# rmcar17/SpectralClusterSupertree

Measured on NVIDIA B200. Metric: construct_supertree wall-time at 10k taxa/1k trees, lower is better.
Workload: dtype f64

## Files before the change

spectralclustersupertree_b200/csrc/common.cuh:

```cuda
#pragma once

#include <cuda_runtime.h>

#include <cstdint>
#include <cstdio>
#include <cstring>
#include <string>
#include <vector>

#include "scs_b200.h"

namespace scs {

constexpr int kMediumMaxDefault = 4096;

struct DeviceBuffer {
    void *ptr = nullptr;
    size_t bytes = 0;
};

enum Slot : int {
    SLOT_TOUR_OFFSETS = 0,
    SLOT_TOUR_TAXON,
    SLOT_TOUR_DEPTH,
// ... 223 lines not shown
int pcg_degree_block(scs_ctx *ctx, int n, int T, RowBlock rows, const double *W_block, double *degree);

int components(scs_ctx *ctx, int n, const uint32_t *bits, int32_t *label, int32_t *n_components_host);

int components_async(scs_ctx *ctx, int n, const uint32_t *bits, int32_t *label, int32_t *count_dev);

int contract(scs_ctx *ctx, int n, const double *W, const uint32_t *adj_bits, const uint32_t *max_bits,
             int32_t *group, int32_t *m_host, double *Wc, double *degree_c);
int contract_with_labels(scs_ctx *ctx, int n, const double *W, const uint32_t *adj_bits, const int32_t *label, int m,
                         int32_t *group, double *Wc, double *degree_c, RowBlock rows = RowBlock());

int spectral_bipartition(scs_ctx *ctx, int m, const double *W, const double *degree, uint64_t seed,
                         int32_t *side, scs_node_stats *stats_host, RowBlock rows = RowBlock());

int normalized_matvec(scs_ctx *ctx, int m, const double *W, const double *isd, const double *x, double *y);

int pcg_build_batch(scs_ctx *ctx, int B, int blocks, int R, int T, int64_t L, int max_n, int max_trees, const MedNode *nodes_dev,
                    const int32_t *tree_node, const int32_t *row_node, const int64_t *leaf_offsets,
                    const int32_t *leaf_taxon, const int32_t *adj_depth, const double *adj_val,
                    const int32_t *root_depth, const double *tree_weight, double *W, int32_t *occ, uint32_t *adj_bits,
                    uint32_t *max_bits, double *degree, int32_t *bad_dev);

constexpr int kMediumMax = kMediumMaxDefault;

int medium_batch(scs_ctx *ctx, int B, const int32_t *node_n, const int32_t *tree_begin, const int32_t *tree_end,
                 const int64_t *part_off, const uint64_t *seeds, int T, int64_t L, const int64_t *leaf_offsets, const int32_t *leaf_taxon,
                 const int32_t *adj_depth, const double *adj_val, const int32_t *root_depth, const double *tree_weight,
                 int contract_edges, int32_t *part_dev, scs_node_stats *stats_host, uint8_t *needs_rerun);

int small_node(scs_ctx *ctx, int n, int contract_edges, const double *W, const uint32_t *adj_bits,
               const uint32_t *max_bits, int32_t *part, scs_node_stats *out_dev, int32_t *group_out,
               double *Wc_out);

int small_batch(scs_ctx *ctx, int num_nodes, const scs_small_node *nodes_dev, const int64_t *leaf_offsets,
                const int32_t *leaf_taxon, const int32_t *adj_depth, const double *adj_val, const int32_t *root_depth,
                const double *tree_weight, int contract_edges, int32_t *part_dev, scs_node_stats *stats_dev,
                int32_t *bad_dev, int absolute_offsets = 0);

int small_cycles(scs_ctx *ctx, unsigned long long *out2, int reset);

int node_split(scs_ctx *ctx, int n, int T, int64_t L, const int64_t *leaf_offsets, const int32_t *leaf_taxon,
               const int32_t *adj_depth, const double *adj_val, const int32_t *root_depth,
               const double *tree_weight, int contract_edges, uint64_t seed, int32_t *part_dev,
               int32_t *part_host, scs_node_stats *stats);

bool shard_applies(const scs_ctx *ctx, int n);
int shard_barrier(scs_ctx *ctx);
int shard_push(scs_ctx *ctx, size_t offset, size_t bytes);
struct ShardMatvecTicket {
    unsigned long long epoch;
    size_t vec_offset;
    unsigned long long timeout_ns;
};
ShardMatvecTicket shard_next_matvec(scs_ctx *ctx);
int node_split_sharded(scs_ctx *ctx, int n, int T, int64_t L, const int64_t *leaf_offsets, const int32_t *leaf_taxon,
                       const int32_t *adj_depth, const double *adj_val, const int32_t *root_depth,
                       const double *tree_weight, int contract_edges, uint64_t seed, int32_t *part_dev,
                       int32_t *part_host, scs_node_stats *stats);

}
```

spectralclustersupertree_b200/csrc/devdriver.cu:

```cuda

#include "common.cuh"

#include <algorithm>
#include <chrono>
#include <cmath>
#include <cstdio>
#include <cstdlib>
#include <thread>

#include "devforest.cuh"
#include "driver.hpp"
#include "forest.hpp"

struct scs_device_forest {
    scs::DevForest trees;
    int weighting = 0;
    int num_taxa = 0;
    std::vector<int32_t> taxa;
    int64_t first_tree_nodes = 0, pair_visits = 0, leaves = 0;
    scs_ctx *owner = nullptr;
};

namespace scs {

// ... 361 lines not shown
                     std::vector<size_t> &reruns) {
        const DevForest &forest = current();
        const int B = static_cast<int>(medium.size());
        std::vector<int32_t> node_n(B), tree_begin(B), tree_end(B);
        std::vector<int64_t> part_off(B);
        std::vector<uint64_t> seeds(B);
        for (int b = 0; b < B; ++b) {
            const Job &job = wave[medium[b]];
            node_n[b] = static_cast<int32_t>(job.taxa.size());
            tree_begin[b] = job.where.tree_begin;
            tree_end[b] = job.where.tree_begin + job.where.trees;
            part_off[b] = splits[b].part_at;
            seeds[b] = node_seed(seed_, job.taxa[0], job.taxa.size());
        }
        std::vector<scs_node_stats> stats(B);
        std::vector<uint8_t> rerun(B, 0);
        int rc = medium_batch(ctx, B, node_n.data(), tree_begin.data(), tree_end.data(), part_off.data(), seeds.data(),
                              static_cast<int>(forest.trees), forest.leaves, forest.leaf_off.as<int64_t>(),
                              tours_.leaf_taxon.as<int32_t>(), tours_.adj_depth.as<int32_t>(), tours_.adj_val.as<double>(),
                              tours_.root_depth.as<int32_t>(), forest.weight.as<double>(), contract_, part_dev_.as<int32_t>(),
                              stats.data(), rerun.data());
        if (rc) return rc;
        for (int b = 0; b < B; ++b) {
            splits[b].stats = stats[b];
            if (rerun[b]) reruns.push_back(static_cast<size_t>(b));
        }
        return SCS_OK;
    }

    int split_small(scs_ctx *ctx, std::vector<Job> &wave, const std::vector<size_t> &small, Split *splits) {
        const DevForest &forest = current();
        const int B = static_cast<int>(small.size());
        std::vector<scs_small_node> desc(B);
        for (int b = 0; b < B; ++b) {
            const Job &job = wave[small[b]];
            desc[b].n = static_cast<int32_t>(job.taxa.size());
            desc[b].num_trees = job.where.trees;
            desc[b].leaf_base = job.where.leaf_begin;
            desc[b].tree_base = job.where.tree_begin;
            desc[b].vertex_base = splits[b].part_at;
        }
        int rc;
        const size_t bytes = sizeof(scs_small_node) * static_cast<size_t>(B);
        scs_small_node *desc_dev;
        if ((rc = reserve_as(ctx, SLOT_MED_NODES, static_cast<size_t>(B), &desc_dev))) return rc;
        void *pin_v;
        if ((rc = reserve_pinned(ctx, bytes + sizeof(scs_node_stats) * static_cast<size_t>(B) + 512, &pin_v))) return rc;
        unsigned char *pin = static_cast<unsigned char *>(pin_v);
        std::memcpy(pin, desc.data(), bytes);
        SCS_CUDA(ctx, cudaMemcpyAsync(desc_dev, pin, bytes, cudaMemcpyHostToDevice, ctx->stream));
        ctx->h2d_bytes += static_cast<int64_t>(bytes);
        scs_node_stats *stats_dev;
        if ((rc = reserve_as(ctx, SLOT_NODE_STATS, static_cast<size_t>(B), &stats_dev))) return rc;
        rc = small_batch(ctx, B, desc_dev, forest.leaf_off.as<int64_t>(), tours_.leaf_taxon.as<int32_t>(),
                         tours_.adj_depth.as<int32_t>(), tours_.adj_val.as<double>(), tours_.root_depth.as<int32_t>(),
                         forest.weight.as<double>(), contract_, part_dev_.as<int32_t>(), stats_dev, flags_dev_.as<int32_t>(), 1);
        if (rc) return rc;
        scs_node_stats *stats_pin = reinterpret_cast<scs_node_stats *>(pin + ((bytes + 255) & ~static_cast<size_t>(255)));
        SCS_CUDA(ctx, cudaMemcpyAsync(stats_pin, stats_dev, sizeof(scs_node_stats) * static_cast<size_t>(B), cudaMemcpyDeviceToHost,
                                       ctx->stream));
        SCS_CUDA(ctx, cudaStreamSynchronize(ctx->stream));
        ctx->d2h_bytes += static_cast<int64_t>(sizeof(scs_node_stats)) * B;
        for (int b = 0; b < B; ++b) splits[b].stats = stats_pin[b];
        return SCS_OK;
    }

    int plan_children(std::vector<Job> &wave, std::vector<Split> &splits, std::vector<Job> &next) {
        const int J = static_cast<int>(wave.size());
        std::vector<int32_t> job_tree_begin(static_cast<size_t>(J) + 1, 0), job_parts(J, 0), job_part_base(J, 0);
        for (int j = 0; j < J; ++j) job_tree_begin[j] = wave[j].where.tree_begin;
        job_tree_begin[J] = static_cast<int32_t>(current().trees);
        std::sort(splits.begin(), splits.end(), [](const Split &a, const Split &b) { return a.job < b.job; });
        struct Pending {
            int32_t parent_slot;
            bool parent_shared, stays;
            std::vector<int32_t> members;
        };
        std::vector<Pending> pending;
        std::vector<int32_t> part_newjob;
        std::vector<int32_t> start, members, cursor;
        for (Split &s : splits) {
            const Job &job = wave[s.job];
            const std::vector<int32_t> &taxa = job.taxa;
            const int n = static_cast<int>(taxa.size());
            const int parts = s.stats.n_components != 1 ? s.stats.n_components : 2;
            const int32_t *part = part_.data() + s.part_at;
            if (record_) {
// ... 195 lines not shown
```

spectralclustersupertree_b200/csrc/driver.cu:

```cuda

#include "common.cuh"

#include <algorithm>
#include <chrono>
#include <cstdio>
#include <cstdlib>
#include <cmath>
#include <memory>
#include <thread>

#include <omp.h>

#include "forest.hpp"
#include "driver.hpp"

namespace scs {

namespace {

constexpr int kMaxWorkers = 16;
int node_workers() {
    static const int value = [] {
        const char *env = std::getenv("SCS_NODE_WORKERS");
        const int v = env ? std::atoi(env) : 8;
// ... 68 lines not shown
    int32_t *tax() const { return reinterpret_cast<int32_t *>(base + o_tax); }
    int32_t *dep() const { return reinterpret_cast<int32_t *>(base + o_dep); }
    int32_t *root() const { return reinterpret_cast<int32_t *>(base + o_root); }
};

int small_stage(scs_ctx *ctx, int num_nodes, int64_t L_total, int64_t T_total, SmallStage *st) {
    const size_t nB = static_cast<size_t>(num_nodes), nL = static_cast<size_t>(L_total), nT = static_cast<size_t>(T_total);
    st->o_nodes = 0;
    st->o_off = st->o_nodes + nB * sizeof(scs_small_node);
    st->o_val = st->o_off + (nT + nB) * sizeof(int64_t);
    st->o_w = st->o_val + nL * sizeof(double);
    st->o_tax = st->o_w + nT * sizeof(double);
    st->o_dep = st->o_tax + nL * sizeof(int32_t);
    st->o_root = st->o_dep + nL * sizeof(int32_t);
    st->total = st->o_root + nT * sizeof(int32_t) + 64;
    if (ctx->pinned_io_bytes < st->total) {
        if (ctx->pinned_io) {
            SCS_CUDA(ctx, cudaStreamSynchronize(ctx->stream));
            SCS_CUDA(ctx, cudaFreeHost(ctx->pinned_io));
            ctx->pinned_io = nullptr;
            ctx->pinned_io_bytes = 0;
        }
        const size_t want = 2 * st->total + 4096;
        SCS_CUDA(ctx, cudaMallocHost(&ctx->pinned_io, want));
        ctx->pinned_io_bytes = want;
    }
    st->base = static_cast<unsigned char *>(ctx->pinned_io);
    return SCS_OK;
}

int small_run(scs_ctx *ctx, int num_nodes, const SmallStage &st, int contract_edges, int32_t *part,
              scs_node_stats *stats) {
    int64_t N_total = 0;
    const scs_small_node *nodes = st.nodes();
    for (int b = 0; b < num_nodes; ++b) {
        if (nodes[b].n < 1 || nodes[b].n > kSmallNode || nodes[b].num_trees < 0)
            return fail(ctx, SCS_ERR_INVALID, "small batch: node size out of range");
        if (nodes[b].num_trees > kSmallMaxTrees)
            return fail(ctx, SCS_ERR_INVALID, "small batch: more than 65 535 source trees at a node (use scs_node_split_*)");
        N_total += nodes[b].n;
    }
    const size_t nB = static_cast<size_t>(num_nodes);
    unsigned char *dev;
    int rc;
    if ((rc = reserve_as(ctx, SLOT_TOUR_OFFSETS, st.total, &dev))) return rc;
    SCS_CUDA(ctx, cudaMemcpyAsync(dev, st.base, st.total - 64, cudaMemcpyHostToDevice, ctx->stream));
    ctx->h2d_bytes += static_cast<int64_t>(st.total - 64);

    int32_t *part_dev, *bad_dev;
    scs_node_stats *stats_dev;
    if ((rc = reserve_as(ctx, SLOT_PART, static_cast<size_t>(N_total), &part_dev))) return rc;
    if ((rc = reserve_as(ctx, SLOT_NODE_STATS, nB, &stats_dev))) return rc;
    if ((rc = reserve_as(ctx, SLOT_SCALARS, 64, &bad_dev))) return rc;
    SCS_CUDA(ctx, cudaMemsetAsync(bad_dev, 0, sizeof(int32_t), ctx->stream));
    rc = small_batch(ctx, num_nodes, reinterpret_cast<const scs_small_node *>(dev + st.o_nodes),
                     reinterpret_cast<const int64_t *>(dev + st.o_off), reinterpret_cast<const int32_t *>(dev + st.o_tax),
                     reinterpret_cast<const int32_t *>(dev + st.o_dep), reinterpret_cast<const double *>(dev + st.o_val),
                     reinterpret_cast<const int32_t *>(dev + st.o_root), reinterpret_cast<const double *>(dev + st.o_w),
                     contract_edges, part_dev, stats_dev, bad_dev);
    if (rc) return rc;
    void *pin_v;
    if ((rc = reserve_pinned(ctx, 64, &pin_v))) return rc;
    SCS_CUDA(ctx, cudaMemcpyAsync(part, part_dev, sizeof(int32_t) * N_total, cudaMemcpyDeviceToHost, ctx->stream));
    SCS_CUDA(ctx, cudaMemcpyAsync(stats, stats_dev, sizeof(scs_node_stats) * nB, cudaMemcpyDeviceToHost, ctx->stream));
    SCS_CUDA(ctx, cudaMemcpyAsync(pin_v, bad_dev, sizeof(int32_t), cudaMemcpyDeviceToHost, ctx->stream));
    SCS_CUDA(ctx, cudaStreamSynchronize(ctx->stream));
    ctx->d2h_bytes += static_cast<int64_t>(sizeof(int32_t) * N_total + sizeof(scs_node_stats) * nB);
    if (*static_cast<int32_t *>(pin_v) != 0) return fail(ctx, SCS_ERR_INPUT, "leaf tour: taxon id out of range");
    for (int b = 0; b < num_nodes; ++b)
        if (stats[b].solver == -1) {
            stats[b].solver = 0;
            return fail(ctx, SCS_ERR_TOO_SMALL, "spectral step on a graph contracted to one vertex");
        }
    return SCS_OK;
}

class Driver {
  public:
    Driver(scs_ctx *ctx, int weighting, int contract_edges, uint64_t seed, bool record, int rank, int world,
           scs_supertree *out)
        : ctx_(ctx), weighting_(weighting), contract_(contract_edges), seed_(seed), record_(record), rank_(rank),
          world_(world), out_(*out) {}

    int run(const scs_forest *root) {
        num_taxa_ = scs_forest_num_taxa(root);
        scratch_.resize(static_cast<size_t>(std::max(scs_host_threads(), kMaxWorkers)));
        for (Scratch &sc : scratch_) sc.reset(num_taxa_);
        std::vector<Task> wave, next;
// ... 665 lines not shown
                               const int32_t *adj_depth, const double *adj_val, const int32_t *root_depth,
                               const double *tree_weight, int contract_edges, int32_t *part, scs_node_stats *stats) {
    if (!ctx || num_nodes < 0 || !nodes || !part || !stats || L_total < 0 || T_total < 0) return SCS_ERR_INVALID;
    if (num_nodes == 0) return SCS_OK;
    cudaSetDevice(ctx->device);
    SmallStage st;
    int rc = small_stage(ctx, num_nodes, L_total, T_total, &st);
    if (rc) return rc;
    const size_t nB = static_cast<size_t>(num_nodes), nL = static_cast<size_t>(L_total), nT = static_cast<size_t>(T_total);
    std::memcpy(st.nodes(), nodes, nB * sizeof(scs_small_node));
    std::memcpy(st.off(), leaf_offsets, (nT + nB) * sizeof(int64_t));
    if (nL) {
        std::memcpy(st.val(), adj_val, nL * sizeof(double));
        std::memcpy(st.tax(), leaf_taxon, nL * sizeof(int32_t));
        std::memcpy(st.dep(), adj_depth, nL * sizeof(int32_t));
    }
    if (nT) {
        std::memcpy(st.w(), tree_weight, nT * sizeof(double));
        std::memcpy(st.root(), root_depth, nT * sizeof(int32_t));
    }
    return small_run(ctx, num_nodes, st, contract_edges, part, stats);
}

int scs_nodes_split_small_dev(scs_ctx *ctx, int num_nodes, const scs_small_node *nodes_dev,
                              const int64_t *leaf_offsets_dev, const int32_t *leaf_taxon_dev,
                              const int32_t *adj_depth_dev, const double *adj_val_dev, const int32_t *root_depth_dev,
                              const double *tree_weight_dev, int contract_edges, int32_t *part_dev,
                              scs_node_stats *stats_dev) {
    if (!ctx || num_nodes < 0 || !nodes_dev || !part_dev || !stats_dev) return SCS_ERR_INVALID;
    cudaSetDevice(ctx->device);
    int32_t *bad_dev;
    int rc;
    if ((rc = reserve_as(ctx, SLOT_SCALARS, 64, &bad_dev))) return rc;
    return small_batch(ctx, num_nodes, nodes_dev, leaf_offsets_dev, leaf_taxon_dev, adj_depth_dev, adj_val_dev,
                       root_depth_dev, tree_weight_dev, contract_edges, part_dev, stats_dev, bad_dev);
}

int scs_supertree_build_sharded(scs_ctx *ctx, const scs_forest *forest, int weighting, int contract_edges,
                                uint64_t seed, int record_nodes, int rank, int world, scs_supertree **out) {
    if (!ctx || !forest || !out || weighting < 0 || weighting > 3 || world < 1 || rank < 0 || rank >= world)
        return SCS_ERR_INVALID;
    *out = nullptr;
    cudaSetDevice(ctx->device);
    std::unique_ptr<scs_supertree> result(new scs_supertree());
    int rc;
    const ShardState &sh = ctx->shard;
    const bool cooperative = world > 1 && sh.connected && sh.world == world && sh.rank == rank;
    if (ctx->device_forest && (world == 1 || cooperative)) {
        const scs_device_forest *resident = nullptr;
        const auto t0 = std::chrono::steady_clock::now();
        if ((rc = device_forest_refresh(ctx, forest, weighting, cooperative, &resident))) return rc;
        const auto t1 = std::chrono::steady_clock::now();
        rc = run_device_driver(ctx, resident, contract_edges, seed, record_nodes != 0, rank, world, result.get());
        const auto t2 = std::chrono::steady_clock::now();
        if (std::getenv("SCS_DRIVER_TRACE")) {
            auto ms = [](auto a, auto b) { return 1e3 * std::chrono::duration<double>(b - a).count(); };
            std::fprintf(stderr, "[scs build] rank %d: forest to the device %.2f ms, recursion %.2f ms, release %.2f ms\n", rank,
                         ms(t0, t1), ms(t1, t2), ms(t2, std::chrono::steady_clock::now()));
        }
    } else {
        Driver driver(ctx, weighting, contract_edges, seed, record_nodes != 0, rank, world, result.get());
        rc = driver.run(forest);
    }
    if (rc) return rc;
    if (world > 1 && result->shared_prefix == 0) result->shared_prefix = static_cast<int64_t>(result->parent.size());
    *out = result.release();
    return SCS_OK;
// ... 113 lines not shown
```

spectralclustersupertree_b200/csrc/pcg.cu:

```cuda

#include "common.cuh"

namespace scs {

namespace {

constexpr int kRowThreads = 512;
constexpr int kWarps = kRowThreads / 32;
constexpr size_t kRowsStaticSmem = 16 * 1024;

struct BatchView {
    const MedNode *nodes = nullptr;
    const int32_t *tree_node = nullptr;
    const int32_t *row_node = nullptr;
};

__global__ void pcg_index_leaves(int n, int T, int64_t L, const int64_t *__restrict__ leaf_offsets,
                                 const int32_t *__restrict__ leaf_taxon, int32_t *__restrict__ leaf_tree,
                                 int32_t *__restrict__ occ, int32_t *__restrict__ bad, BatchView batch) {
    int64_t g = blockIdx.x * static_cast<int64_t>(blockDim.x) + threadIdx.x;
    if (g >= L) return;
    int lo = 0, hi = T;
    while (hi - lo > 1) {
        int mid = (lo + hi) >> 1;
// ... 65 lines not shown

__global__ void pcg_sort_inverse(int row0, const int32_t *__restrict__ row_ptr, const int32_t *__restrict__ inv,
                                 int32_t *__restrict__ inv_sorted) {
    __shared__ int32_t stage[1024];
    const int a = row0 + blockIdx.x;
    const int base = row_ptr[a];
    const int cnt = row_ptr[a + 1] - base;
    for (int i0 = 0; i0 < cnt; i0 += blockDim.x) {
        const int i = i0 + threadIdx.x;
        const int32_t mine = i < cnt ? inv[base + i] : 0;
        int rank = 0;
        for (int j0 = 0; j0 < cnt; j0 += 1024) {
            const int len = min(1024, cnt - j0);
            __syncthreads();
            for (int j = threadIdx.x; j < len; j += blockDim.x) stage[j] = inv[base + j0 + j];
            __syncthreads();
            if (i < cnt)
                for (int j = 0; j < len; ++j) rank += stage[j] < mine;
        }
        if (i < cnt) inv_sorted[base + rank] = mine;
    }
}

struct __align__(16) LinkEntry {
    int32_t next_right, next_left;
    double val;
};
constexpr int32_t kNone = -1;
constexpr int32_t kRootLevel = -2;

__global__ void __launch_bounds__(256)
pcg_tour_links(int n, const int64_t *__restrict__ leaf_offsets, const int32_t *__restrict__ adj_depth,
               const double *__restrict__ adj_val, const int32_t *__restrict__ root_depth,
               LinkEntry *__restrict__ links) {
    extern __shared__ int32_t link_smem[];
    const int t = blockIdx.x;
    const int64_t tb = leaf_offsets[t];
    const int m = static_cast<int>(leaf_offsets[t + 1] - tb) - 1;
    if (m <= 0 || m >= n) return;
    const int32_t *D = adj_depth + tb;
    const int nb1 = (m + 31) >> 5, nb2 = (nb1 + 31) >> 5;
    int32_t *B1 = link_smem, *B2 = link_smem + nb1;
    const int lane = threadIdx.x & 31;
    for (int i0 = (threadIdx.x >> 5) << 5; i0 < m; i0 += blockDim.x) {
        int v = i0 + lane < m ? D[i0 + lane] : INT32_MAX;
#pragma unroll
        for (int off = 16; off > 0; off >>= 1) v = min(v, __shfl_xor_sync(0xffffffffu, v, off));
        if (lane == 0) B1[i0 >> 5] = v;
    }
    __syncthreads();
    for (int b0 = (threadIdx.x >> 5) << 5; b0 < nb1; b0 += blockDim.x) {
        int v = b0 + lane < nb1 ? B1[b0 + lane] : INT32_MAX;
#pragma unroll
        for (int off = 16; off > 0; off >>= 1) v = min(v, __shfl_xor_sync(0xffffffffu, v, off));
        if (lane == 0) B2[b0 >> 5] = v;
    }
    __syncthreads();
    const int rd = root_depth[t];
    for (int i = threadIdx.x; i < m; i += blockDim.x) {
        const int d = D[i];
        LinkEntry e;
        e.val = adj_val[tb + i];
        if (d == rd) {
            e.next_right = e.next_left = kRootLevel;
            links[tb + i] = e;
            continue;
        }
        int j = i + 1;
        {
// ... 957 lines not shown
    if ((rc = reserve_as(ctx, SLOT_LEAF_TREE, static_cast<size_t>(L) + 1, &leaf_tree))) return rc;
    if ((rc = reserve_as(ctx, SLOT_ROW_PTR, static_cast<size_t>(n) + 1, &row_ptr))) return rc;
    if ((rc = reserve_as(ctx, SLOT_CURSOR, static_cast<size_t>(n), &cursor))) return rc;
    if ((rc = reserve_as(ctx, SLOT_INV, static_cast<size_t>(L) + 1, &inv))) return rc;
    if ((rc = reserve_as(ctx, SLOT_INV_SORTED, static_cast<size_t>(L) + 1, &inv_sorted))) return rc;
    if ((rc = reserve_as(ctx, SLOT_SCALARS, 64, &scalars))) return rc;

    SCS_CUDA(ctx, cudaMemsetAsync(occ, 0, sizeof(int32_t) * n, ctx->stream));
    SCS_CUDA(ctx, cudaMemsetAsync(cursor, 0, sizeof(int32_t) * n, ctx->stream));
    SCS_CUDA(ctx, cudaMemsetAsync(scalars, 0, sizeof(int32_t) * 64, ctx->stream));
    if (L > 0) {
        pcg_index_leaves<<<ceil_div(L, 256), 256, 0, ctx->stream>>>(n, T, L, leaf_offsets, leaf_taxon, leaf_tree, occ,
                                                                   scalars, BatchView());
        SCS_LAUNCHED(ctx, "pcg_index_leaves");
    }
    if ((rc = exclusive_scan(ctx, n, occ, row_ptr))) return rc;
    if (L > 0) {
        pcg_fill_inverse<<<ceil_div(L, 256), 256, 0, ctx->stream>>>(n, L, leaf_taxon, leaf_tree, row_ptr, cursor, inv,
                                                                   BatchView());
        SCS_LAUNCHED(ctx, "pcg_fill_inverse");
        if (nrows > 0) {
            pcg_sort_inverse<<<nrows, 128, 0, ctx->stream>>>(row0, row_ptr, inv, inv_sorted);
            SCS_LAUNCHED(ctx, "pcg_sort_inverse");
        }
    }
    LinkEntry *links;
    if ((rc = reserve_as(ctx, SLOT_LINKS, static_cast<size_t>(L > 0 ? L : 1), &links))) return rc;
    if (L > 0 && T > 0) {
        const int nb1 = ceil_div(n, 32), nb2 = ceil_div(nb1, 32);
        const size_t link_smem = sizeof(int32_t) * (static_cast<size_t>(nb1) + nb2 + 2);
        if (link_smem > 48 * 1024)
            SCS_CUDA(ctx, cudaFuncSetAttribute(pcg_tour_links, cudaFuncAttributeMaxDynamicSharedMemorySize,
                                               static_cast<int>(link_smem)));
        pcg_tour_links<<<T, 256, link_smem, ctx->stream>>>(n, leaf_offsets, adj_depth, adj_val, root_depth, links);
        SCS_LAUNCHED(ctx, "pcg_tour_links");
    }

    const bool narrow = T < 65536;
    const size_t per_col = sizeof(double) + (narrow ? sizeof(uint16_t) : sizeof(int32_t));
    BucketShape bs;
    bs.warps_log2 = 4;
    const int warps = 1 << bs.warps_log2;
    bs.cols_per_chunk = chunk_columns(ctx, n, T);
    const int nchunks = ceil_div(n, bs.cols_per_chunk);
    bs.buckets = nchunks * warps;
    const int stride = ceil_div(bs.cols_per_chunk, warps) | 1;
    const size_t smem = static_cast<size_t>(stride) * warps * per_col + 16;
    if ((rc = reserve_as(ctx, SLOT_DEGREE_PART, static_cast<size_t>(n) * nchunks, &degree_part))) return rc;
    if (nrows == 0) return SCS_OK;

    const bool packed = n <= 65535 && !ctx->wide_entries;
    const size_t cells = static_cast<size_t>(T) * bs.buckets;
    if (cells + 1 >= (1ull << 31)) return fail(ctx, SCS_ERR_INVALID, "pcg_build: too many tree buckets");
    int32_t *bucket_ptr;
    void *entries;
    if ((rc = reserve_as(ctx, SLOT_BUCKET_PTR, cells + 2, &bucket_ptr))) return rc;
    if ((rc = reserve(ctx, SLOT_ENTRIES, (static_cast<size_t>(L) + 1) * (packed ? 4 : 8), &entries))) return rc;
    const bool tri = !rows.sharded() && C == nullptr && !ctx->full_rows;
    const bool half = rows.sharded() && rows.half_window && C == nullptr && !ctx->full_rows;
    int32_t *start16 = nullptr;
    if (tri && (rc = reserve_as(ctx, SLOT_START16, (static_cast<size_t>(L) + 1) * kWarps, &start16))) return rc;
    if ((rc = build_buckets(ctx, n, T, L, bs, stride, packed, leaf_offsets, leaf_taxon, bucket_ptr, entries, start16, scalars,
                            BatchView())))
        return rc;
    LeafStairs *stairs;
    if ((rc = reserve_as(ctx, SLOT_BUCKET_COUNT, static_cast<size_t>(L) + 1, &stairs))) return rc;
    if (L > 0) {
// ... 38 lines not shown
        !row_node || !W || !occ || !adj_bits || !degree || !bad_dev)
        return fail(ctx, SCS_ERR_INVALID, "pcg_build_batch: bad argument");
    BatchView batch;
    batch.nodes = nodes_dev;
    batch.tree_node = tree_node;
    batch.row_node = row_node;
    int32_t *leaf_tree, *row_ptr, *cursor, *inv, *inv_sorted;
    int rc;
    if ((rc = reserve_as(ctx, SLOT_LEAF_TREE, static_cast<size_t>(L) + 1, &leaf_tree))) return rc;
    if ((rc = reserve_as(ctx, SLOT_ROW_PTR, static_cast<size_t>(R) + 1, &row_ptr))) return rc;
    if ((rc = reserve_as(ctx, SLOT_CURSOR, static_cast<size_t>(R), &cursor))) return rc;
    if ((rc = reserve_as(ctx, SLOT_INV, static_cast<size_t>(L) + 1, &inv))) return rc;
    if ((rc = reserve_as(ctx, SLOT_INV_SORTED, static_cast<size_t>(L) + 1, &inv_sorted))) return rc;
    SCS_CUDA(ctx, cudaMemsetAsync(occ, 0, sizeof(int32_t) * R, ctx->stream));
    SCS_CUDA(ctx, cudaMemsetAsync(cursor, 0, sizeof(int32_t) * R, ctx->stream));
    if (L > 0) {
        pcg_index_leaves<<<ceil_div(L, 256), 256, 0, ctx->stream>>>(max_n, T, L, leaf_offsets, leaf_taxon, leaf_tree, occ,
                                                                   bad_dev, batch);
        SCS_LAUNCHED(ctx, "pcg_index_leaves");
    }
    if ((rc = exclusive_scan(ctx, R, occ, row_ptr))) return rc;
    if (L > 0) {
        pcg_fill_inverse<<<ceil_div(L, 256), 256, 0, ctx->stream>>>(max_n, L, leaf_taxon, leaf_tree, row_ptr, cursor, inv,
                                                                   batch);
        SCS_LAUNCHED(ctx, "pcg_fill_inverse");
        pcg_sort_inverse<<<R, 128, 0, ctx->stream>>>(0, row_ptr, inv, inv_sorted);
        SCS_LAUNCHED(ctx, "pcg_sort_inverse");
    }
    LinkEntry *links;
    if ((rc = reserve_as(ctx, SLOT_LINKS, static_cast<size_t>(L > 0 ? L : 1), &links))) return rc;
    if (L > 0 && T > 0) {
        const int nb1 = ceil_div(max_n + 1, 32), nb2 = ceil_div(nb1, 32);
        const size_t link_smem = sizeof(int32_t) * (static_cast<size_t>(nb1) + nb2 + 2);
        pcg_tour_links<<<T, 256, link_smem, ctx->stream>>>(max_n + 1, leaf_offsets, adj_depth, adj_val, root_depth, links);
        SCS_LAUNCHED(ctx, "pcg_tour_links");
    }
    const bool narrow = max_trees < 65536;
    const size_t per_col = sizeof(double) + (narrow ? sizeof(uint16_t) : sizeof(int32_t));
    BucketShape bs;
    bs.warps_log2 = 4;
    const int warps = 1 << bs.warps_log2;
    bs.cols_per_chunk = ceil_div(max_n, 32) * 32;
    bs.buckets = warps;
    const int stride = ceil_div(bs.cols_per_chunk, warps) | 1;
    const size_t smem = static_cast<size_t>(stride) * warps * per_col + 16;
    const size_t cells = static_cast<size_t>(T) * bs.buckets;
    if (cells + 1 >= (1ull << 31)) return fail(ctx, SCS_ERR_INVALID, "pcg_build_batch: too many tree buckets");
    int32_t *bucket_ptr;
    void *entries;
    if ((rc = reserve_as(ctx, SLOT_BUCKET_PTR, cells + 2, &bucket_ptr))) return rc;
    if ((rc = reserve(ctx, SLOT_ENTRIES, (static_cast<size_t>(L) + 1) * 4, &entries))) return rc;
    int32_t *start16 = nullptr;
    if (!ctx->full_rows && (rc = reserve_as(ctx, SLOT_START16, (static_cast<size_t>(L) + 1) * kWarps, &start16))) return rc;
    if ((rc = build_buckets(ctx, max_n, T, L, bs, stride, true, leaf_offsets, leaf_taxon, bucket_ptr, entries, start16, bad_dev,
                            batch)))
        return rc;
    LeafStairs *stairs;
    if ((rc = reserve_as(ctx, SLOT_BUCKET_COUNT, static_cast<size_t>(L) + 1, &stairs))) return rc;
    if (L > 0) {
        pcg_leaf_stairs<<<ceil_div(L, kStairsLeaves), 2 * kStairsLeaves, 0, ctx->stream>>>(max_n, L, leaf_offsets, leaf_tree, links, tree_weight,
                                                                      stairs, bad_dev, batch);
        SCS_LAUNCHED(ctx, "pcg_leaf_stairs");
    }
    if (!ctx->full_rows) {
        if (narrow)
            rc = launch_rows<uint16_t, false, uint32_t, true>(ctx, R, 0, R, 0, bs, stride, 1, smem, leaf_offsets, links,
                                                              tree_weight, leaf_tree, row_ptr, inv_sorted, occ, bucket_ptr,
// ... 23 lines not shown
```

spectralclustersupertree_b200/csrc/small.cu:

```cuda

#include "common.cuh"

namespace scs {

namespace {

constexpr int kN = kSmallNode;
constexpr int kThreads = 256;
constexpr double kGapTie = 1e-7;
constexpr double kMarginTie = 1e-9;

struct SmallShared {
    double A[kN][kN + 1];
    double V[kN][kN + 1];
    double B[kN][kN + 1];
    unsigned short cnt[kN][kN];
    int occ[kN];
    int tour_taxon[kN], tour_depth[kN];
    double tour_val[kN];
    double cs[kN / 2][2];
    double deg[kN], isd[kN], q0[kN], u[kN], sorted[kN];
    unsigned long long adj[kN], mx[kN], reach[kN];
    int label[kN], group[kN], member_of[kN], side[kN];
    double red[kThreads / 32 + 1];
    int ired[4];
};

__device__ __forceinline__ double block_sum_small(double v, double *red) {
#pragma unroll
    for (int off = 16; off > 0; off >>= 1) v += __shfl_down_sync(0xffffffffu, v, off);
    __syncthreads();
    if ((threadIdx.x & 31) == 0) red[threadIdx.x >> 5] = v;
    __syncthreads();
    if (threadIdx.x == 0) {
        double s = 0.0;
        for (int w = 0; w < kThreads / 32; ++w) s += red[w];
        red[kThreads / 32] = s;
    }
    __syncthreads();
    return red[kThreads / 32];
}

__device__ void closure(int n, const unsigned long long *rows, unsigned long long *reach, int *label) {
    const int v = threadIdx.x;
    if (v < n) reach[v] = rows[v] | (1ull << v);
    __syncthreads();
    for (int round = 0; round < 6; ++round) {
        unsigned long long acc = 0;
        if (v < n) {
            unsigned long long bits = reach[v];
            acc = bits;
            while (bits) {
                const int b = __ffsll(static_cast<long long>(bits)) - 1;
                bits &= bits - 1;
                acc |= reach[b];
            }
        }
        __syncthreads();
        if (v < n) reach[v] = acc;
        __syncthreads();
    }
    if (v < n) label[v] = __ffsll(static_cast<long long>(reach[v])) - 1;
    __syncthreads();
}

__device__ void small_finish(SmallShared &S, int n, int contract_edges, int32_t *__restrict__ part,
                             scs_node_stats *__restrict__ out, int32_t *__restrict__ group_out,
                             double *__restrict__ Wc_out) {
    const int tid = threadIdx.x;
    const double nan_v = __longlong_as_double(0x7ff8000000000000ll);

    closure(n, S.adj, S.reach, S.label);
    if (tid == 0) {
        int count = 0;
        for (int v = 0; v < n; ++v) {
            S.member_of[v] = count;
            count += S.label[v] == v;
        }
        S.ired[0] = count;
    }
    __syncthreads();
    const int ncomp = S.ired[0];
    if (tid == 0) {
        out->n_components = ncomp;
        out->contracted_size = n;
        out->spectral_ran = 0;
        out->solver = 0;
        out->matvecs = 0;
        out->restarts = 0;
        out->tie_flag = 0;
        out->kmeans_stable_splits = 0;
        out->eig[0] = 0.0;
        out->eig[1] = nan_v;
        out->eig[2] = nan_v;
        out->residual = nan_v;
        out->margin = nan_v;
        out->kmeans_runner_up = 0.0;
    }
    if (ncomp != 1) {
// ... 249 lines not shown
        if (theta1 - theta2 < kGapTie) flag |= 1;
        if (!(margin >= kMarginTie)) flag |= 2;
        if (S.ired[2]) flag |= 8;
        if (stable > 1) flag |= 16;
        out->tie_flag = flag;
    }
    __syncthreads();
    const double threshold = S.red[3];
    if (tid < m) S.side[tid] = S.u[tid] >= threshold ? 1 : 0;
    __syncthreads();
    if (tid < n) part[tid] = S.side[S.group[tid]];

    if (tid < m) {
        double acc = 0.0;
        for (int j = 0; j < m; ++j)
            if (j != tid) acc += S.isd[tid] * S.B[tid][j] * S.isd[j] * S.V[j][col];
        acc -= theta1 * S.V[tid][col];
        S.deg[tid] = acc * acc;
    }
    __syncthreads();
    if (tid == 0) {
        double rr = 0.0;
        for (int i = 0; i < m; ++i) rr += S.deg[i];
        out->residual = sqrt(rr);
    }
}

__global__ void __launch_bounds__(kThreads)
small_node_kernel(int n, int words, int contract_edges, const double *__restrict__ W,
                  const uint32_t *__restrict__ adj_bits, const uint32_t *__restrict__ max_bits,
                  int32_t *__restrict__ part, scs_node_stats *__restrict__ out,
                  int32_t *__restrict__ group_out, double *__restrict__ Wc_out) {
    extern __shared__ __align__(16) unsigned char raw[];
    SmallShared &S = *reinterpret_cast<SmallShared *>(raw);
    const int tid = threadIdx.x;
    for (int e = tid; e < n * n; e += kThreads) S.A[e / n][e % n] = W[e];
    if (tid < n) {
        unsigned long long a = adj_bits[static_cast<size_t>(tid) * words];
        unsigned long long m = max_bits ? max_bits[static_cast<size_t>(tid) * words] : 0ull;
        if (words > 1) {
            a |= static_cast<unsigned long long>(adj_bits[static_cast<size_t>(tid) * words + 1]) << 32;
            if (max_bits) m |= static_cast<unsigned long long>(max_bits[static_cast<size_t>(tid) * words + 1]) << 32;
        }
        S.adj[tid] = a;
        S.mx[tid] = m;
    }
    __syncthreads();
    small_finish(S, n, contract_edges, part, out, group_out, Wc_out);
}

__device__ unsigned long long g_small_cycles[2];

__global__ void __launch_bounds__(kThreads)
small_batch_kernel(const scs_small_node *__restrict__ nodes, const int64_t *__restrict__ leaf_offsets,
                   const int32_t *__restrict__ leaf_taxon, const int32_t *__restrict__ adj_depth,
                   const double *__restrict__ adj_val, const int32_t *__restrict__ root_depth,
                   const double *__restrict__ tree_weight, int contract_edges, int32_t *__restrict__ part,
                   scs_node_stats *__restrict__ stats, int32_t *__restrict__ bad, int absolute_offsets) {
    extern __shared__ __align__(16) unsigned char raw[];
    SmallShared &S = *reinterpret_cast<SmallShared *>(raw);
    const int tid = threadIdx.x;
    const scs_small_node node = nodes[blockIdx.x];
    const int n = node.n;
    const long long clock_start = clock64();
    if (node.num_trees > kSmallMaxTrees || n < 1 || n > kN) {
        if (tid == 0) {
            *bad = 1;
            stats[blockIdx.x].solver = -1;
        }
        return;
    }
    for (int e = tid; e < n * n; e += kThreads) {
        S.A[e / n][e % n] = 0.0;
        S.cnt[e / n][e % n] = 0;
    }
    if (tid < n) S.occ[tid] = 0;
    __syncthreads();
    const int64_t *offs = leaf_offsets + node.tree_base + (absolute_offsets ? 0 : blockIdx.x);
    const int64_t leaf_base = absolute_offsets ? 0 : node.leaf_base;
    for (int t = 0; t < node.num_trees; ++t) {
        const int64_t tb = leaf_base + offs[t];
        const int k = static_cast<int>(offs[t + 1] - offs[t]);
        const double w = tree_weight[node.tree_base + t];
        const int rd = root_depth[node.tree_base + t];
        if (k > n) {
            if (tid == 0) *bad = 1;
            continue;
        }
        if (tid < k) {
            const int a = leaf_taxon[tb + tid];
            S.tour_taxon[tid] = a;
            S.tour_depth[tid] = adj_depth[tb + tid];
            S.tour_val[tid] = adj_val[tb + tid];
            if (a < 0 || a >= n) *bad = 1;
        }
        __syncthreads();
        const int i = tid & (kN - 1), q = tid >> 6;
        if (i < k) {
            const int a = S.tour_taxon[i];
            if (a >= 0 && a < n) {
                if (q == 0) S.occ[a] += 1;
                int best_depth = 0x7fffffff, best_idx = i;
                for (int j = i + 1; j < k; ++j) {
                    const int d = S.tour_depth[j - 1];
                    if (d < best_depth) { best_depth = d; best_idx = j - 1; }
                    if (best_depth == rd) break;
                    if (((j - i - 1) & 3) != q) continue;
                    const int b = S.tour_taxon[j];
                    if (b < 0 || b >= n) continue;
                    const int lo = min(a, b), hi = max(a, b);
                    S.A[lo][hi] = __dadd_rn(S.A[lo][hi], __dmul_rn(S.tour_val[best_idx], w));
                    S.cnt[lo][hi] += 1;
                }
            }
        }
        __syncthreads();
    }
    for (int e = tid; e < n * n; e += kThreads) {
        const int r = e / n, c = e % n;
        if (r > c) {
            S.A[r][c] = S.A[c][r];
            S.cnt[r][c] = S.cnt[c][r];
        }
    }
    __syncthreads();
    if (tid < n) {
        unsigned long long a = 0, m = 0;
        const int occ_a = S.occ[tid];
        for (int b = 0; b < n; ++b) {
            const int c = S.cnt[tid][b];
            if (c > 0) {
                a |= 1ull << b;
                if (c == max(occ_a, S.occ[b])) m |= 1ull << b;
            }
        }
        S.adj[tid] = a;
        S.mx[tid] = contract_edges ? m : 0ull;
    }
    __syncthreads();
    const long long clock_built = clock64();
    small_finish(S, n, contract_edges, part + node.vertex_base, stats + blockIdx.x, nullptr, nullptr);
    if (tid == 0) {
        atomicAdd(&g_small_cycles[0], static_cast<unsigned long long>(clock_built - clock_start));
        atomicAdd(&g_small_cycles[1], static_cast<unsigned long long>(clock64() - clock_built));
    }
}

}

int small_node(scs_ctx *ctx, int n, int contract_edges, const double *W, const uint32_t *adj_bits,
               const uint32_t *max_bits, int32_t *part, scs_node_stats *out_dev, int32_t *group_out,
               double *Wc_out) {
    if (n < 1 || n > kSmallNode) return fail(ctx, SCS_ERR_INVALID, "small_node: size out of range");
    const size_t smem = sizeof(SmallShared);
    if (!ctx->small_configured) {
        SCS_CUDA(ctx, cudaFuncSetAttribute(small_node_kernel, cudaFuncAttributeMaxDynamicSharedMemorySize,
                                           static_cast<int>(smem)));
        ctx->small_configured = true;
    }
    small_node_kernel<<<1, kThreads, smem, ctx->stream>>>(n, scs_bit_words(n), contract_edges, W, adj_bits,
                                                         contract_edges ? max_bits : nullptr, part, out_dev, group_out,
                                                         Wc_out);
    SCS_LAUNCHED(ctx, "small_node_kernel");
    return SCS_OK;
}

int small_cycles(scs_ctx *ctx, unsigned long long *out2, int reset) {
    SCS_CUDA(ctx, cudaStreamSynchronize(ctx->stream));
    SCS_CUDA(ctx, cudaMemcpyFromSymbol(out2, g_small_cycles, 2 * sizeof(unsigned long long)));
    if (reset) {
        const unsigned long long zero[2] = {0, 0};
        SCS_CUDA(ctx, cudaMemcpyToSymbol(g_small_cycles, zero, sizeof(zero)));
    }
    return SCS_OK;
}

int small_batch(scs_ctx *ctx, int num_nodes, const scs_small_node *nodes_dev, const int64_t *leaf_offsets,
                const int32_t *leaf_taxon, const int32_t *adj_depth, const double *adj_val, const int32_t *root_depth,
                const double *tree_weight, int contract_edges, int32_t *part_dev, scs_node_stats *stats_dev,
                int32_t *bad_dev, int absolute_offsets) {
    if (num_nodes <= 0) return SCS_OK;
    const size_t smem = sizeof(SmallShared);
    if (!ctx->batch_configured) {
        SCS_CUDA(ctx, cudaFuncSetAttribute(small_batch_kernel, cudaFuncAttributeMaxDynamicSharedMemorySize,
                                           static_cast<int>(smem)));
        ctx->batch_configured = true;
    }
    small_batch_kernel<<<num_nodes, kThreads, smem, ctx->stream>>>(nodes_dev, leaf_offsets, leaf_taxon, adj_depth,
                                                                  adj_val, root_depth, tree_weight, contract_edges,
                                                                  part_dev, stats_dev, bad_dev, absolute_offsets);
    SCS_LAUNCHED(ctx, "small_batch_kernel");
    return SCS_OK;
}

}
```

Measured before the change: 0.06489.

## Template small batch kernel on node size and stage many trees per sync

Templates the small-node batch kernel on N, adding a 32-wide variant chosen when every node in the batch has at most 32 taxa. That variant uses a smaller shared footprint (allowing two blocks per SM) and stages up to 128 trees' tours into shared memory per chunk. Tree offsets, weights and root depths are loaded once per chunk instead of being read from global memory every tree iteration. Separately, pcg_tour_links now skips trees whose tree_node entry is negative in the batched PCG path. The cost is more template instances and somewhat more complex chunk-boundary logic.

```diff
diff --git a/spectralclustersupertree_b200/csrc/common.cuh b/spectralclustersupertree_b200/csrc/common.cuh
--- a/spectralclustersupertree_b200/csrc/common.cuh
+++ b/spectralclustersupertree_b200/csrc/common.cuh
@@ -279,7 +279,7 @@
                const uint32_t *max_bits, int32_t *part, scs_node_stats *out_dev, int32_t *group_out,
                double *Wc_out);
 
-int small_batch(scs_ctx *ctx, int num_nodes, const scs_small_node *nodes_dev, const int64_t *leaf_offsets,
+int small_batch(scs_ctx *ctx, int num_nodes, int max_n, const scs_small_node *nodes_dev, const int64_t *leaf_offsets,
                 const int32_t *leaf_taxon, const int32_t *adj_depth, const double *adj_val, const int32_t *root_depth,
                 const double *tree_weight, int contract_edges, int32_t *part_dev, scs_node_stats *stats_dev,
                 int32_t *bad_dev, int absolute_offsets = 0);
diff --git a/spectralclustersupertree_b200/csrc/devdriver.cu b/spectralclustersupertree_b200/csrc/devdriver.cu
--- a/spectralclustersupertree_b200/csrc/devdriver.cu
+++ b/spectralclustersupertree_b200/csrc/devdriver.cu
@@ -417,6 +417,7 @@
         const DevForest &forest = current();
         const int B = static_cast<int>(small.size());
         std::vector<scs_small_node> desc(B);
+        int max_n = 0;
         for (int b = 0; b < B; ++b) {
             const Job &job = wave[small[b]];
             desc[b].n = static_cast<int32_t>(job.taxa.size());
@@ -424,6 +425,7 @@
             desc[b].leaf_base = job.where.leaf_begin;
             desc[b].tree_base = job.where.tree_begin;
             desc[b].vertex_base = splits[b].part_at;
+            max_n = std::max(max_n, desc[b].n);
         }
         int rc;
         const size_t bytes = sizeof(scs_small_node) * static_cast<size_t>(B);
@@ -437,7 +439,7 @@
         ctx->h2d_bytes += static_cast<int64_t>(bytes);
         scs_node_stats *stats_dev;
         if ((rc = reserve_as(ctx, SLOT_NODE_STATS, static_cast<size_t>(B), &stats_dev))) return rc;
-        rc = small_batch(ctx, B, desc_dev, forest.leaf_off.as<int64_t>(), tours_.leaf_taxon.as<int32_t>(),
+        rc = small_batch(ctx, B, max_n, desc_dev, forest.leaf_off.as<int64_t>(), tours_.leaf_taxon.as<int32_t>(),
                          tours_.adj_depth.as<int32_t>(), tours_.adj_val.as<double>(), tours_.root_depth.as<int32_t>(),
                          forest.weight.as<double>(), contract_, part_dev_.as<int32_t>(), stats_dev, flags_dev_.as<int32_t>(), 1);
         if (rc) return rc;
diff --git a/spectralclustersupertree_b200/csrc/driver.cu b/spectralclustersupertree_b200/csrc/driver.cu
--- a/spectralclustersupertree_b200/csrc/driver.cu
+++ b/spectralclustersupertree_b200/csrc/driver.cu
@@ -124,6 +124,7 @@
 int small_run(scs_ctx *ctx, int num_nodes, const SmallStage &st, int contract_edges, int32_t *part,
               scs_node_stats *stats) {
     int64_t N_total = 0;
+    int max_n = 0;
     const scs_small_node *nodes = st.nodes();
     for (int b = 0; b < num_nodes; ++b) {
         if (nodes[b].n < 1 || nodes[b].n > kSmallNode || nodes[b].num_trees < 0)
@@ -131,6 +132,7 @@
         if (nodes[b].num_trees > kSmallMaxTrees)
             return fail(ctx, SCS_ERR_INVALID, "small batch: more than 65 535 source trees at a node (use scs_node_split_*)");
         N_total += nodes[b].n;
+        max_n = std::max(max_n, nodes[b].n);
     }
     const size_t nB = static_cast<size_t>(num_nodes);
     unsigned char *dev;
@@ -145,7 +147,7 @@
     if ((rc = reserve_as(ctx, SLOT_NODE_STATS, nB, &stats_dev))) return rc;
     if ((rc = reserve_as(ctx, SLOT_SCALARS, 64, &bad_dev))) return rc;
     SCS_CUDA(ctx, cudaMemsetAsync(bad_dev, 0, sizeof(int32_t), ctx->stream));
-    rc = small_batch(ctx, num_nodes, reinterpret_cast<const scs_small_node *>(dev + st.o_nodes),
+    rc = small_batch(ctx, num_nodes, max_n, reinterpret_cast<const scs_small_node *>(dev + st.o_nodes),
                      reinterpret_cast<const int64_t *>(dev + st.o_off), reinterpret_cast<const int32_t *>(dev + st.o_tax),
                      reinterpret_cast<const int32_t *>(dev + st.o_dep), reinterpret_cast<const double *>(dev + st.o_val),
                      reinterpret_cast<const int32_t *>(dev + st.o_root), reinterpret_cast<const double *>(dev + st.o_w),
@@ -877,7 +879,7 @@
     int32_t *bad_dev;
     int rc;
     if ((rc = reserve_as(ctx, SLOT_SCALARS, 64, &bad_dev))) return rc;
-    return small_batch(ctx, num_nodes, nodes_dev, leaf_offsets_dev, leaf_taxon_dev, adj_depth_dev, adj_val_dev,
+    return small_batch(ctx, num_nodes, kSmallNode, nodes_dev, leaf_offsets_dev, leaf_taxon_dev, adj_depth_dev, adj_val_dev,
                        root_depth_dev, tree_weight_dev, contract_edges, part_dev, stats_dev, bad_dev);
 }
 
diff --git a/spectralclustersupertree_b200/csrc/pcg.cu b/spectralclustersupertree_b200/csrc/pcg.cu
--- a/spectralclustersupertree_b200/csrc/pcg.cu
+++ b/spectralclustersupertree_b200/csrc/pcg.cu
@@ -121,9 +121,10 @@
 __global__ void __launch_bounds__(256)
 pcg_tour_links(int n, const int64_t *__restrict__ leaf_offsets, const int32_t *__restrict__ adj_depth,
                const double *__restrict__ adj_val, const int32_t *__restrict__ root_depth,
-               LinkEntry *__restrict__ links) {
+               const int32_t *__restrict__ tree_node, LinkEntry *__restrict__ links) {
     extern __shared__ int32_t link_smem[];
     const int t = blockIdx.x;
+    if (tree_node && tree_node[t] < 0) return;
     const int64_t tb = leaf_offsets[t];
     const int m = static_cast<int>(leaf_offsets[t + 1] - tb) - 1;
     if (m <= 0 || m >= n) return;
@@ -1147,7 +1148,7 @@
         if (link_smem > 48 * 1024)
             SCS_CUDA(ctx, cudaFuncSetAttribute(pcg_tour_links, cudaFuncAttributeMaxDynamicSharedMemorySize,
                                                static_cast<int>(link_smem)));
-        pcg_tour_links<<<T, 256, link_smem, ctx->stream>>>(n, leaf_offsets, adj_depth, adj_val, root_depth, links);
+        pcg_tour_links<<<T, 256, link_smem, ctx->stream>>>(n, leaf_offsets, adj_depth, adj_val, root_depth, nullptr, links);
         SCS_LAUNCHED(ctx, "pcg_tour_links");
     }
 
@@ -1252,7 +1253,8 @@
     if (L > 0 && T > 0) {
         const int nb1 = ceil_div(max_n + 1, 32), nb2 = ceil_div(nb1, 32);
         const size_t link_smem = sizeof(int32_t) * (static_cast<size_t>(nb1) + nb2 + 2);
-        pcg_tour_links<<<T, 256, link_smem, ctx->stream>>>(max_n + 1, leaf_offsets, adj_depth, adj_val, root_depth, links);
+        pcg_tour_links<<<T, 256, link_smem, ctx->stream>>>(max_n + 1, leaf_offsets, adj_depth, adj_val, root_depth,
+                                                             tree_node, links);
         SCS_LAUNCHED(ctx, "pcg_tour_links");
     }
     const bool narrow = max_trees < 65536;
diff --git a/spectralclustersupertree_b200/csrc/small.cu b/spectralclustersupertree_b200/csrc/small.cu
--- a/spectralclustersupertree_b200/csrc/small.cu
+++ b/spectralclustersupertree_b200/csrc/small.cu
@@ -5,25 +5,38 @@
 
 namespace {
 
-constexpr int kN = kSmallNode;
-constexpr int kThreads = 256;
 constexpr double kGapTie = 1e-7;
 constexpr double kMarginTie = 1e-9;
-
+constexpr int kThreads = 256;
+
+template <int N>
+struct SmallCfg {
+    static constexpr int kLeafThreads = kThreads / N;
+    static constexpr int kStageLeaves = N == 32 ? 512 : N;
+    static constexpr int kStageTrees = N == 32 ? 128 : 8;
+    static constexpr int kMinBlocks = N == 32 ? 2 : 1;
+};
+
+template <int N>
 struct SmallShared {
-    double A[kN][kN + 1];
-    double V[kN][kN + 1];
-    double B[kN][kN + 1];
-    unsigned short cnt[kN][kN];
-    int occ[kN];
-    int tour_taxon[kN], tour_depth[kN];
-    double tour_val[kN];
-    double cs[kN / 2][2];
-    double deg[kN], isd[kN], q0[kN], u[kN], sorted[kN];
-    unsigned long long adj[kN], mx[kN], reach[kN];
-    int label[kN], group[kN], member_of[kN], side[kN];
+    using Cfg = SmallCfg<N>;
+    double A[N][N + 1];
+    double V[N][N + 1];
+    double B[N][N + 1];
+    unsigned short cnt[N][N];
+    int occ[N];
+    int64_t stage_off[Cfg::kStageTrees + 1];
+    double stage_w[Cfg::kStageTrees];
+    int stage_rd[Cfg::kStageTrees];
+    int tour_taxon[Cfg::kStageLeaves], tour_depth[Cfg::kStageLeaves];
+    double tour_val[Cfg::kStageLeaves];
+    double cs[N / 2][2];
+    double deg[N], isd[N], q0[N], u[N], sorted[N];
+    unsigned long long adj[N], mx[N], reach[N];
+    int label[N], group[N], member_of[N], side[N];
     double red[kThreads / 32 + 1];
     int ired[4];
+    int chunk_end;
 };
 
 __device__ __forceinline__ double block_sum_small(double v, double *red) {
@@ -64,7 +77,8 @@
     __syncthreads();
 }
 
-__device__ void small_finish(SmallShared &S, int n, int contract_edges, int32_t *__restrict__ part,
+template <int N>
+__device__ void small_finish(SmallShared<N> &S, int n, int contract_edges, int32_t *__restrict__ part,
                              scs_node_stats *__restrict__ out, int32_t *__restrict__ group_out,
                              double *__restrict__ Wc_out) {
     const int tid = threadIdx.x;
@@ -380,7 +394,7 @@
                   int32_t *__restrict__ part, scs_node_stats *__restrict__ out,
                   int32_t *__restrict__ group_out, double *__restrict__ Wc_out) {
     extern __shared__ __align__(16) unsigned char raw[];
-    SmallShared &S = *reinterpret_cast<SmallShared *>(raw);
+    SmallShared<kSmallNode> &S = *reinterpret_cast<SmallShared<kSmallNode> *>(raw);
     const int tid = threadIdx.x;
     for (int e = tid; e < n * n; e += kThreads) S.A[e / n][e % n] = W[e];
     if (tid < n) {
@@ -399,19 +413,21 @@
 
 __device__ unsigned long long g_small_cycles[2];
 
-__global__ void __launch_bounds__(kThreads)
+template <int N>
+__global__ void __launch_bounds__(kThreads, SmallCfg<N>::kMinBlocks)
 small_batch_kernel(const scs_small_node *__restrict__ nodes, const int64_t *__restrict__ leaf_offsets,
                    const int32_t *__restrict__ leaf_taxon, const int32_t *__restrict__ adj_depth,
                    const double *__restrict__ adj_val, const int32_t *__restrict__ root_depth,
                    const double *__restrict__ tree_weight, int contract_edges, int32_t *__restrict__ part,
                    scs_node_stats *__restrict__ stats, int32_t *__restrict__ bad, int absolute_offsets) {
+    using Cfg = SmallCfg<N>;
     extern __shared__ __align__(16) unsigned char raw[];
-    SmallShared &S = *reinterpret_cast<SmallShared *>(raw);
+    SmallShared<N> &S = *reinterpret_cast<SmallShared<N> *>(raw);
     const int tid = threadIdx.x;
     const scs_small_node node = nodes[blockIdx.x];
     const int n = node.n;
     const long long clock_start = clock64();
-    if (node.num_trees > kSmallMaxTrees || n < 1 || n > kN) {
+    if (node.num_trees > kSmallMaxTrees || n < 1 || n > N) {
         if (tid == 0) {
             *bad = 1;
             stats[blockIdx.x].solver = -1;
@@ -423,47 +439,74 @@
         S.cnt[e / n][e % n] = 0;
     }
     if (tid < n) S.occ[tid] = 0;
-    __syncthreads();
     const int64_t *offs = leaf_offsets + node.tree_base + (absolute_offsets ? 0 : blockIdx.x);
     const int64_t leaf_base = absolute_offsets ? 0 : node.leaf_base;
-    for (int t = 0; t < node.num_trees; ++t) {
-        const int64_t tb = leaf_base + offs[t];
-        const int k = static_cast<int>(offs[t + 1] - offs[t]);
-        const double w = tree_weight[node.tree_base + t];
-        const int rd = root_depth[node.tree_base + t];
-        if (k > n) {
-            if (tid == 0) *bad = 1;
-            continue;
-        }
-        if (tid < k) {
-            const int a = leaf_taxon[tb + tid];
-            S.tour_taxon[tid] = a;
-            S.tour_depth[tid] = adj_depth[tb + tid];
-            S.tour_val[tid] = adj_val[tb + tid];
-            if (a < 0 || a >= n) *bad = 1;
-        }
-        __syncthreads();
-        const int i = tid & (kN - 1), q = tid >> 6;
-        if (i < k) {
-            const int a = S.tour_taxon[i];
-            if (a >= 0 && a < n) {
-                if (q == 0) S.occ[a] += 1;
-                int best_depth = 0x7fffffff, best_idx = i;
-                for (int j = i + 1; j < k; ++j) {
-                    const int d = S.tour_depth[j - 1];
-                    if (d < best_depth) { best_depth = d; best_idx = j - 1; }
-                    if (best_depth == rd) break;
-                    if (((j - i - 1) & 3) != q) continue;
-                    const int b = S.tour_taxon[j];
-                    if (b < 0 || b >= n) continue;
-                    const int lo = min(a, b), hi = max(a, b);
-                    S.A[lo][hi] = __dadd_rn(S.A[lo][hi], __dmul_rn(S.tour_val[best_idx], w));
-                    S.cnt[lo][hi] += 1;
+    const double *weight = tree_weight + node.tree_base;
+    const int *rdepth = root_depth + node.tree_base;
+    const int i = tid & (N - 1), q = tid / N;
+    for (int t0 = 0; t0 < node.num_trees;) {
+        const int nt = min(Cfg::kStageTrees, node.num_trees - t0);
+        if (tid == 0) S.chunk_end = nt;
+        for (int x = tid; x <= nt; x += kThreads) S.stage_off[x] = offs[t0 + x];
+        for (int x = tid; x < nt; x += kThreads) {
+            S.stage_w[x] = weight[t0 + x];
+            S.stage_rd[x] = rdepth[t0 + x];
+        }
+        __syncthreads();
+        for (int x = tid + 1; x <= nt; x += kThreads)
+            if (S.stage_off[x] - S.stage_off[0] > Cfg::kStageLeaves || S.stage_off[x] < S.stage_off[x - 1])
+                atomicMin(&S.chunk_end, x - 1);
+        __syncthreads();
+        int trees = S.chunk_end;
+        int staged = static_cast<int>(S.stage_off[trees] - S.stage_off[0]);
+        if (trees == 0) {
+            trees = 1;
+            staged = 0;
+        }
+        const int64_t first = leaf_base + S.stage_off[0];
+        for (int x = tid; x < staged; x += kThreads) {
+            S.tour_taxon[x] = leaf_taxon[first + x];
+            S.tour_depth[x] = adj_depth[first + x];
+            S.tour_val[x] = adj_val[first + x];
+        }
+        __syncthreads();
+        for (int t = 0; t < trees; ++t) {
+            const int tb = static_cast<int>(S.stage_off[t] - S.stage_off[0]);
+            const int k = static_cast<int>(S.stage_off[t + 1] - S.stage_off[t]);
+            const double w = S.stage_w[t];
+            const int rd = S.stage_rd[t];
+            if (k > n) {
+                if (tid == 0) *bad = 1;
+            } else if (tid < k) {
+                const int a = S.tour_taxon[tb + tid];
+                if (a < 0 || a >= n) *bad = 1;
+            }
+            if (i < k && k <= n) {
+                const int *taxon = S.tour_taxon + tb;
+                const int *depth = S.tour_depth + tb;
+                const double *val = S.tour_val + tb;
+                const int a = taxon[i];
+                if (a >= 0 && a < n) {
+                    if (q == 0) S.occ[a] += 1;
+                    int best_depth = 0x7fffffff, best_idx = i;
+                    for (int j = i + 1; j < k; ++j) {
+                        const int d = depth[j - 1];
+                        if (d < best_depth) { best_depth = d; best_idx = j - 1; }
+                        if (best_depth == rd) break;
+                        if (((j - i - 1) & (Cfg::kLeafThreads - 1)) != q) continue;
+                        const int b = taxon[j];
+                        if (b < 0 || b >= n) continue;
+                        const int lo = min(a, b), hi = max(a, b);
+                        S.A[lo][hi] = __dadd_rn(S.A[lo][hi], __dmul_rn(val[best_idx], w));
+                        S.cnt[lo][hi] += 1;
+                    }
                 }
             }
-        }
-        __syncthreads();
-    }
+            __syncthreads();
+        }
+        t0 += trees;
+    }
+    __syncthreads();
     for (int e = tid; e < n * n; e += kThreads) {
         const int r = e / n, c = e % n;
         if (r > c) {
@@ -500,15 +543,15 @@
                const uint32_t *max_bits, int32_t *part, scs_node_stats *out_dev, int32_t *group_out,
                double *Wc_out) {
     if (n < 1 || n > kSmallNode) return fail(ctx, SCS_ERR_INVALID, "small_node: size out of range");
-    const size_t smem = sizeof(SmallShared);
+    const size_t smem = sizeof(SmallShared<kSmallNode>);
     if (!ctx->small_configured) {
         SCS_CUDA(ctx, cudaFuncSetAttribute(small_node_kernel, cudaFuncAttributeMaxDynamicSharedMemorySize,
                                            static_cast<int>(smem)));
         ctx->small_configured = true;
     }
-    small_node_kernel<<<1, kThreads, smem, ctx->stream>>>(n, scs_bit_words(n), contract_edges, W, adj_bits,
-                                                         contract_edges ? max_bits : nullptr, part, out_dev, group_out,
-                                                         Wc_out);
+    small_node_kernel<<<1, kThreads, smem, ctx->stream>>>(
+        n, scs_bit_words(n), contract_edges, W, adj_bits, contract_edges ? max_bits : nullptr, part, out_dev, group_out,
+        Wc_out);
     SCS_LAUNCHED(ctx, "small_node_kernel");
     return SCS_OK;
 }
@@ -523,20 +566,27 @@
     return SCS_OK;
 }
 
-int small_batch(scs_ctx *ctx, int num_nodes, const scs_small_node *nodes_dev, const int64_t *leaf_offsets,
+int small_batch(scs_ctx *ctx, int num_nodes, int max_n, const scs_small_node *nodes_dev, const int64_t *leaf_offsets,
                 const int32_t *leaf_taxon, const int32_t *adj_depth, const double *adj_val, const int32_t *root_depth,
                 const double *tree_weight, int contract_edges, int32_t *part_dev, scs_node_stats *stats_dev,
                 int32_t *bad_dev, int absolute_offsets) {
     if (num_nodes <= 0) return SCS_OK;
-    const size_t smem = sizeof(SmallShared);
     if (!ctx->batch_configured) {
-        SCS_CUDA(ctx, cudaFuncSetAttribute(small_batch_kernel, cudaFuncAttributeMaxDynamicSharedMemorySize,
-                                           static_cast<int>(smem)));
+        SCS_CUDA(ctx, cudaFuncSetAttribute(small_batch_kernel<32>, cudaFuncAttributeMaxDynamicSharedMemorySize,
+                                           static_cast<int>(sizeof(SmallShared<32>))));
+        SCS_CUDA(ctx, cudaFuncSetAttribute(small_batch_kernel<kSmallNode>, cudaFuncAttributeMaxDynamicSharedMemorySize,
+                                           static_cast<int>(sizeof(SmallShared<kSmallNode>))));
         ctx->batch_configured = true;
     }
-    small_batch_kernel<<<num_nodes, kThreads, smem, ctx->stream>>>(nodes_dev, leaf_offsets, leaf_taxon, adj_depth,
-                                                                  adj_val, root_depth, tree_weight, contract_edges,
-                                                                  part_dev, stats_dev, bad_dev, absolute_offsets);
+    if (max_n <= 32)
+        small_batch_kernel<32><<<num_nodes, kThreads, sizeof(SmallShared<32>), ctx->stream>>>(
+            nodes_dev, leaf_offsets, leaf_taxon, adj_depth, adj_val, root_depth, tree_weight, contract_edges, part_dev,
+            stats_dev, bad_dev, absolute_offsets);
+    else
+        small_batch_kernel<kSmallNode><<<num_nodes, kThreads, sizeof(SmallShared<kSmallNode>),
+                                         ctx->stream>>>(nodes_dev, leaf_offsets, leaf_taxon, adj_depth, adj_val, root_depth,
+                                                        tree_weight, contract_edges, part_dev, stats_dev, bad_dev,
+                                                        absolute_offsets);
     SCS_LAUNCHED(ctx, "small_batch_kernel");
     return SCS_OK;
 }
```

After: 0.06320 (median of 6 runs). 1.03x faster.
